# Oujidejihe/PG2024-Data-Parallel-Ray-Tracing

Measured on NVIDIA B200. Metric: Mrays/s, higher is better.
Workload: dtype f32

## Files before the change

include/dprt_types.h:

```cpp
#ifndef DPRT_TYPES_H
#define DPRT_TYPES_H

#include <stdint.h>
#include <stddef.h>

#ifdef __cplusplus
extern "C" {
#endif

#define DPRT_DEFAULT_MAX_COUNT 3
#define DPRT_DEFAULT_SHADOW_PATH_COUNT 4
#define DPRT_EPSILON 1e-3f
#define DPRT_MAX_WORLD 32
#define DPRT_MAX_SCENE_OBJECTS 64
#define DPRT_MAX_LIGHTS 64
#define DPRT_MAX_MATERIALS 256

typedef struct dprt_path_record {
    float    origin[3];
    float    direction[3];
    float    tMax;
    float    throughput[3];
    int32_t  pixelIndex;
    int32_t  shadowPathID;
// ... 127 lines not shown
    int64_t rays_shade;
    int64_t rays_shadow;
    int64_t rays_secondary;
    int64_t nn_queries;
    int64_t paths_sent_offrank;
    int64_t exchange_iters;
    int64_t kernel_launches;
    int64_t bytes_alltoall;
    int64_t rays_shade_cached;
    int64_t rays_walked;
    int64_t walked_traverse;
    int64_t walked_shade;
    int64_t walked_shadow;
    int64_t walked_secondary;
    int64_t paths_partitioned;
} dprt_stats;

enum dprt_buffer_id {
    DPRT_BUF_PATHS = 0,
    DPRT_BUF_TRANSFER = 1,
    DPRT_BUF_TRANSFER_OFFSET = 2,
    DPRT_BUF_DIRECT = 3,
    DPRT_BUF_ENV = 4,
    DPRT_BUF_NN_INPUT = 5,
    DPRT_BUF_NN_QUERY = 6,
    DPRT_BUF_NN_PACKED_INPUT = 7,
    DPRT_BUF_NN_PACKED_QUERY = 8,
    DPRT_BUF_SCENE_OFFSET = 9,
    DPRT_BUF_PRED = 10,
    DPRT_BUF_OCCLUSION = 11,
// ... 49 lines not shown
```

pg2024-data-parallel-ray-tracing_b200/csrc/dprt_api.cu:

```cuda
#include <cuda_runtime.h>
#include <dlfcn.h>
#include <nccl.h>

#include <algorithm>
#include <atomic>
#include <cstdio>
#include <cstring>
#include <memory>
#include <string>
#include <thread>
#include <vector>

#include "dprt.h"
#include "dprt_internal.cuh"
#include "bvh_build.h"
#include "scene_flatten.h"
#include "mlp.cuh"
#include "p2p_exchange.cuh"

using namespace dprt;

struct dprt_bvh8 { Bvh8 b; };

constexpr int kDevStats = 2 + DPRT_STAGE_COUNT;

namespace {

std::string g_create_error;

std::atomic<int> g_streams[64];
int max_connections() {
    const char* e = getenv("CUDA_DEVICE_MAX_CONNECTIONS");
    const int v = e ? atoi(e) : 8;
    return v < 1 ? 1 : (v > 32 ? 32 : v);
}

struct NcclApi {
    void* handle = nullptr;
    ncclResult_t (*GetUniqueId)(ncclUniqueId*) = nullptr;
// ... 102 lines not shown
    P2PPlan* d_plan = nullptr;
    P2PHostPlan* h_plan = nullptr;
    P2PHostPlan* d_hplan = nullptr;
    uint32_t p2pSeq = 0;
    std::vector<void*> ipcOpened;
    int32_t* d_secLive = nullptr;
    int secDirty = 0;
    bool nnScratchDirty = false;
    uint32_t epoch = 1;
    int32_t* d_queue = nullptr;
    cudaStream_t aux = nullptr;
    cudaEvent_t evShade = nullptr, evAux = nullptr;
    int32_t* d_queue_aux = nullptr;
    bool auxPending = false;
    int auxGuardBase = 0;
    float* d_image = nullptr;
    float* d_image_sum = nullptr;
    int32_t* d_gather = nullptr;
    int32_t* h_pinned = nullptr;
    void* d_flush = nullptr; size_t flush_bytes = 0;
    void* d_io = nullptr; size_t io_bytes = 0;
    HitRec* d_rayPark = nullptr; size_t rayParkCount = 0;
    int pathSize = 0, shadowPathSize = 0;
    int sample = 0;
    int queryTotal = 0;
    int queryWhich = 0;
    std::vector<int> h_sceneOffset;
    bool histFresh = false;
    bool qhistFresh = false;
    std::vector<int> h_offsets;
// ... 355 lines not shown
    CK(cudaSetDevice(ctx->device));
    CK(cudaStreamSynchronize(ctx->stream));
    CK(cudaGetLastError());
    return 0;
}
int dprt_get_stats(const dprt_ctx* ctx, dprt_stats* out) {
    if (!ctx || !out) return DPRT_ERR_INVALID;
    *out = ctx->stats;
    if (ctx->d_cacheHits) {
        unsigned long long v[kDevStats] = {0};
        if (cudaSetDevice(ctx->device) != cudaSuccess || cudaStreamSynchronize(ctx->stream) != cudaSuccess ||
            cudaMemcpy(v, ctx->d_cacheHits, sizeof(v), cudaMemcpyDeviceToHost) != cudaSuccess) return DPRT_ERR_CUDA;
        out->rays_shade_cached = (int64_t)v[0]; out->rays_walked = (int64_t)v[1];
        out->walked_traverse = (int64_t)v[2 + DPRT_STAGE_TRAVERSE]; out->walked_shade = (int64_t)v[2 + DPRT_STAGE_SHADE];
        out->walked_shadow = (int64_t)v[2 + DPRT_STAGE_SHADOW_TRACE]; out->walked_secondary = (int64_t)v[2 + DPRT_STAGE_SECONDARY_TRACE];
    }
    return 0;
}
int dprt_reset_stats(dprt_ctx* ctx) {
    if (!ctx) return DPRT_ERR_INVALID;
    ctx->stats = dprt_stats{};
    cudaSetDevice(ctx->device);
    resolve_pending(ctx);
    for (int i = 0; i < DPRT_STAGE_COUNT; i++) { ctx->stageMs[i] = 0.0; ctx->stageLaunches[i] = 0; }
    if (ctx->d_counters) CK(cudaMemsetAsync(ctx->d_counters, 0, 2 * DPRT_STAGE_COUNT * sizeof(unsigned long long), ctx->stream));
    if (ctx->d_cacheHits) CK(cudaMemsetAsync(ctx->d_cacheHits, 0, kDevStats * sizeof(unsigned long long), ctx->stream));
    return 0;
}

int dprt_stage_profile(dprt_ctx* ctx, int enable) {
// ... 350 lines not shown
    if (recv_offset) recv_offset[W] = (int32_t)roff;
    if (recv_total) *recv_total = roff;
    if (all_local) *all_local = offdiag == 0;
    return 0;
}

int dprt_exchange(dprt_ctx* ctx, int* done) {
    if (!ctx) return DPRT_ERR_INVALID;
    CK(cudaSetDevice(ctx->device));
    const int W = ctx->world, me = ctx->rank;
    const size_t R = sizeof(dprt_path_record);
    StageScope sc_(ctx, DPRT_STAGE_EXCHANGE);
    if (W == 1) {
        int r = read_offsets(ctx); if (r) return r;
        const int cnt = ctx->h_offsets[1];
        if (cnt > 0) CK(cudaMemcpyAsync(ctx->hp.paths, ctx->hp.transfer, cnt * R, cudaMemcpyDeviceToDevice, ctx->stream));
        ctx->pathSize = cnt; ctx->stats.paths_partitioned += cnt;
        if (done) *done = 1;
        ctx->stats.exchange_iters++;
        return 0;
    }
    if (!ctx->comm) return fail(ctx, DPRT_ERR_STATE, "dprt_exchange on a multi-rank context without an NCCL communicator");
    NK(g_nccl.AllGather(ctx->hp.transferOffset, ctx->d_gather, W + 1, ncclInt32, ctx->comm, ctx->stream));
    CK(cudaMemcpyAsync(ctx->h_pinned, ctx->d_gather, sizeof(int32_t) * W * (W + 1), cudaMemcpyDeviceToHost, ctx->stream));
    CK(cudaStreamSynchronize(ctx->stream));
    const int32_t* M = ctx->h_pinned;
    ctx->h_offsets.assign(M + me * (W + 1), M + (me + 1) * (W + 1));
    ctx->stats.paths_partitioned += ctx->h_offsets[W];
    std::vector<int32_t> sendCnt(W), recvOff(W + 1, 0), recvCnt(W);
    int64_t recvTotal64 = 0; int allLocal = 0;
    if (dprt_plan_exchange(M, W, me, sendCnt.data(), recvOff.data(), recvCnt.data(), &recvTotal64, &allLocal))
// ... 56 lines not shown
        ctx->stats.exchange_iters++;
    }
    if (done) *done = offdiag == 0;
    return 0;
}

int dprt_shade(dprt_ctx* ctx) {
    if (!ctx) return DPRT_ERR_INVALID;
    CK(cudaSetDevice(ctx->device));
    if (ctx->hp.lightCount < 1) return fail(ctx, DPRT_ERR_STATE, "no lights set");
    ctx->shadowPathSize = ctx->cfg.shadowPathCount * ctx->pathSize;
    const int w = ctx->dirtyIdx == 0 ? 1 : 0;
    ctx->hp.livePixel = ctx->d_live[w]; ctx->liveCount[w] = ctx->pathSize; ctx->shadeIdx = w;
    sync_params(ctx);
    StageScope sc_(ctx, DPRT_STAGE_SHADE, ctx->pathSize > 0);
    launch_shade(ctx->hp, ctx->pathSize, ctx->stream);
    ctx->stats.kernel_launches += trace_kernels_per_stage() * (ctx->pathSize > 0);
    ctx->stats.rays_shade += ctx->pathSize;
    ctx->epoch++;
    ctx->histFresh = false;
    CK(cudaGetLastError());
    return 0;
}

int dprt_reset_nn(dprt_ctx* ctx) {
    if (!ctx) return DPRT_ERR_INVALID;
    CK(cudaSetDevice(ctx->device));
    const bool nnAll = ctx->nnScratchDirty || (ctx->cfg.proxyMode && ctx->dirtyIdx == -2);
    if (nnAll) {
        CK(cudaMemsetAsync(ctx->hp.occlusion, 0, ctx->buf_bytes[DPRT_BUF_OCCLUSION], ctx->stream));
        CK(cudaMemsetAsync(ctx->hp.contribution, 0, ctx->buf_bytes[DPRT_BUF_CONTRIBUTION], ctx->stream));
        ctx->nnScratchDirty = false;
// ... 13 lines not shown
        ctx->stats.kernel_launches += ctx->liveCount[ctx->dirtyIdx] > 0;
    }
    ctx->dirtyIdx = -1;
    CK(cudaMemsetAsync(ctx->hp.queryHist, 0, 64 * sizeof(int32_t), ctx->stream));
    ctx->qhistFresh = false;
    return 0;
}

int dprt_shadow_trace(dprt_ctx* ctx) {
    if (!ctx) return DPRT_ERR_INVALID;
    CK(cudaSetDevice(ctx->device));
    sync_params(ctx);
    CK(cudaMemsetAsync(ctx->hp.queryHist, 0, 64 * sizeof(int32_t), ctx->stream));
    StageScope sc_(ctx, DPRT_STAGE_SHADOW_TRACE, ctx->shadowPathSize > 0);
    launch_shadow_trace(ctx->hp, ctx->shadowPathSize, ctx->stream);
    ctx->stats.kernel_launches += trace_kernels_per_stage() * (ctx->shadowPathSize > 0);
    ctx->stats.rays_shadow += ctx->shadowPathSize;
    if (ctx->shadowPathSize > 0)
        ctx->dirtyIdx = (ctx->shadeIdx >= 0 && (ctx->dirtyIdx == -1 || ctx->dirtyIdx == ctx->shadeIdx)) ? ctx->shadeIdx : -2;
    ctx->qhistFresh = true; ctx->queryWhich = 0;
    CK(cudaGetLastError());
    return 0;
}

int dprt_secondary_trace(dprt_ctx* ctx) {
    if (!ctx) return DPRT_ERR_INVALID;
    CK(cudaSetDevice(ctx->device));
    if (!ctx->cfg.proxyMode) return fail(ctx, DPRT_ERR_STATE, "secondary stage needs proxyMode=1");
    sync_params(ctx);
    CK(cudaMemsetAsync(ctx->hp.queryHist, 0, 64 * sizeof(int32_t), ctx->stream));
    StageScope sc_(ctx, DPRT_STAGE_SECONDARY_TRACE, ctx->pathSize > 0);
// ... 537 lines not shown
    int r;
    if (bounce > 0 && ctx->cfg.proxyMode) {
        if ((r = dprt_reset_nn(ctx))) return r;
        if ((r = dprt_secondary_ray_module(ctx))) return r;
    }
    return 0;
}
int bounce_post(dprt_ctx* ctx) {
    int r;
    if ((r = dprt_shade(ctx))) return r;
    if ((r = dprt_reset_nn(ctx))) return r;
    return dprt_shadow_ray_module(ctx);
}
}

int dprt_render_sample(dprt_ctx* ctx, int sample) {
    if (!ctx) return DPRT_ERR_INVALID;
    int r;
    if ((r = dprt_begin_sample(ctx, sample))) return r;
    if ((r = dprt_path_gen(ctx))) return r;
    const bool overlap = ctx->aux && !ctx->profile;
    for (int bounce = 0; bounce <= ctx->cfg.bounces; bounce++) {
        if ((r = bounce_pre(ctx, bounce))) return r;
        if ((r = dprt_primary_ray_module(ctx))) return r;
        if (!overlap) { if ((r = bounce_post(ctx))) return r; continue; }
        if ((r = join_aux(ctx))) return r;
        if ((r = dprt_shade(ctx))) return r;
        CK(cudaEventRecord(ctx->evShade, ctx->stream));
        cudaStream_t mainStream = ctx->stream; int32_t* mainQueue = ctx->hp.traceQueue;
        ctx->stream = ctx->aux; ctx->hp.traceQueue = ctx->d_queue_aux;
        cudaError_t ce = cudaStreamWaitEvent(ctx->aux, ctx->evShade, 0);
        r = ce != cudaSuccess ? DPRT_ERR_CUDA : dprt_reset_nn(ctx);
        if (!r) r = dprt_shadow_ray_module(ctx);
        if (!r && cudaEventRecord(ctx->evAux, ctx->aux) != cudaSuccess) r = DPRT_ERR_CUDA;
        ctx->stream = mainStream; ctx->hp.traceQueue = mainQueue;
        if (r) return r;
        ctx->auxPending = true; ctx->auxGuardBase = ctx->pathSize;
    }
    return join_aux(ctx);
}

int dprt_render_sample_group(dprt_ctx** ctxs, int W, int sample) {
    if (!ctxs || W < 1) return DPRT_ERR_INVALID;
    int r;
    for (int k = 0; k < W; k++) {
        if ((r = dprt_begin_sample(ctxs[k], sample))) return r;
        if ((r = dprt_path_gen(ctxs[k]))) return r;
    }
    const int bounces = ctxs[0]->cfg.bounces;
    bool deque = true;
    for (int k = 0; k < W; k++) deque = deque && ctxs[k] && deque_enabled(ctxs[k]) && ctxs[k]->world == W && ctxs[k]->rank == k;
    const char* pg = getenv("DPRT_P2P_GROUP");
    bool p2p = deque && W > 1 && W <= 8 && pg && pg[0] == '1';
    if (p2p && !ctxs[0]->p2pGroup) { if ((r = p2p_connect_group(ctxs, W))) return r; }
// ... 274 lines not shown
```

pg2024-data-parallel-ray-tracing_b200/csrc/dprt_internal.cuh:

```cuda
#pragma once
#include <cuda_runtime.h>
#include <stdint.h>
#include "dprt_types.h"
#include "dprt_math.cuh"

namespace dprt {

struct DevObject {
    int32_t nodeID;
    int32_t isProxy;
    float   aabbMin[3];
    float   aabbMax[3];
    float   maxLength;
    float   w2o[12];
    const uint4*  nodes;
    const float4* tris;
    const float*  normals;
};

struct HitRec {
    float   t;
    int32_t prim;
    int32_t tri;
    int32_t obj;
// ... 45 lines not shown
    HitRec*  hitCache;
    uint32_t hitEpoch;
    unsigned long long* cacheHits;
    int32_t  splitL;
    int32_t* secLive;
    int32_t* livePixel;
    const DevTexture* textures;
    const int32_t*    matTex;
    DevTexture        envMap;
    float             envRotation;
};

void launch_path_gen(const DevParams& p, int n, cudaStream_t stream);
void launch_traverse(const DevParams& p, int n, cudaStream_t stream);
void launch_shade(const DevParams& p, int n, cudaStream_t stream);
void launch_shadow_trace(const DevParams& p, int nShadow, cudaStream_t stream);
void launch_secondary_trace(const DevParams& p, int n, cudaStream_t stream);
int trace_kernels_per_stage();
size_t trace_scratch_bytes();
void launch_trace_closest(const DevObject* objects, int sceneSize, const DevTexture* textures, const int32_t* matTex, const dprt_ray* rays,
                          dprt_hit* hits, int64_t n, int32_t* queue, unsigned long long* counters, HitRec* park, cudaStream_t stream);

void launch_train_features(const DevObject* obj, const dprt_ray* rays, const dprt_hit* hits, int64_t n, float* features,
                           float* labels, cudaStream_t stream);

void launch_precom_features(const DevObject* obj, dprt_ray* rays, int64_t n, float* features, float* t_aabb, cudaStream_t stream);
void launch_precom_labels(const DevObject* obj, const dprt_hit* hits, const float* t_aabb, int64_t n, float* labels, uint8_t* valid,
                          cudaStream_t stream);

int spec_texture_sample(const float* rgba, int width, int height, const float* u, const float* v, int64_t n, int clampV, float* out4);
int spec_env_lookup(const float* rgba, int width, int height, float rotationOffset, const float* dirs3, int64_t n, float* out3);
// ... 33 lines not shown
```

pg2024-data-parallel-ray-tracing_b200/csrc/kernels.cu:

```cuda
#include "dprt_internal.cuh"
#include <algorithm>
#include <cstdlib>
#include "bvh_traverse.cuh"

namespace dprt {

namespace {

constexpr int kBlock = 128;

struct PathRegs {
    V3 origin, direction; float tMax; V3 throughput;
    int pixelIndex, shadowPathID; uint32_t visitedMask; int currentNode, targetNode; uint32_t flags;
};
constexpr uint32_t F_SHADOW = 1u, F_DELTA = 1u << 8, F_VALID = 1u << 16, F_HIT = 1u << 24;

DPRT_D PathRegs load_path(const dprt_path_record* p) {
    const float4* q = reinterpret_cast<const float4*>(p);
    float4 a = q[0], b = q[1], c = q[2], d = q[3];
    PathRegs r;
    r.origin = v3(a.x, a.y, a.z); r.direction = v3(a.w, b.x, b.y); r.tMax = b.z;
    r.throughput = v3(b.w, c.x, c.y);
    r.pixelIndex = __float_as_int(c.z); r.shadowPathID = __float_as_int(c.w);
    r.visitedMask = __float_as_uint(d.x); r.currentNode = __float_as_int(d.y);
// ... 84 lines not shown
    const dprt_ray* rays; dprt_hit* rayHits;
    int32_t* hitPrim;
    int32_t* queue;
    unsigned long long* counters;
    int refill;
    int triVote;
    uint32_t prmtMagic;
    uint32_t* coopPool;
    int coop;
    int nodesPerStep;
    HitRec* hitCache; uint32_t epoch; unsigned long long* cacheHits;
    int tailBudget;
    int32_t* parkList;
    HitRec* park;
    const DevTexture* textures; const int32_t* matTex;
};

constexpr int kParkCapacity = 148 * 8 * 128 + 4096;

DPRT_D int next_object(const TraceArgs& a, int from, uint32_t skipMask) {
    for (int k = from; k < a.sceneSize; k++) {
        const DevObject& ob = a.objects[k];
        if (ob.isProxy) continue;
        if ((skipMask >> ob.nodeID) & 1u) continue;
        return k;
    }
    return a.sceneSize;
}


// ... 2 lines not shown
    const bool hit = s.hitTri >= 0;
    if (MODE == TM_TRAVERSE || MODE == TM_SECONDARY || MODE == TM_SHADE) {
        float4* h = reinterpret_cast<float4*>(a.hits + idx);
        h[0] = make_float4(s.tbest, __int_as_float(hit ? s.hitPrim : -1), __int_as_float(s.hitTri), __int_as_float(s.hitObj));
        h[1] = make_float4(s.ha, s.hb, 0.f, 0.f);
    } else if (MODE == TM_SHADOW) {
        if (hit) {
            flags = (flags | F_HIT) & ~F_VALID;
            reinterpret_cast<uint32_t*>(a.recs + idx)[15] = flags;
        }
    } else {
        reinterpret_cast<float2*>(a.rayHits)[idx] = make_float2(s.tbest, __int_as_float(hit ? s.hitPrim : -1));
    }
}

template <int MODE>
DPRT_D bool trace_load_ray(const TraceArgs& a, int my, V3& o, V3& d, float& tmin, float& tmax, uint32_t& flags, uint32_t& skipMask, bool& retry) {
    tmin = DPRT_EPSILON; skipMask = 0u; retry = false; flags = 0u;
    if (MODE == TM_RAYS) {
        const float4 r0 = __ldg(reinterpret_cast<const float4*>(a.rays) + 2 * (size_t)my);
        const float4 r1 = __ldg(reinterpret_cast<const float4*>(a.rays) + 2 * (size_t)my + 1);
        o = v3(r0.x, r0.y, r0.z); tmin = r0.w; d = v3(r1.x, r1.y, r1.z); tmax = r1.w;
        return true;
    }
    const float4* q = reinterpret_cast<const float4*>(a.recs + my);
    const float4 q0 = q[0], q1 = q[1], q3 = q[3];
    o = v3(q0.x, q0.y, q0.z); d = v3(q0.w, q1.x, q1.y); tmax = q1.z;
    flags = __float_as_uint(q3.w);
    if (MODE == TM_TRAVERSE) skipMask = __float_as_uint(q3.x);
    if (MODE == TM_SHADE) {
// ... 2 lines not shown
            tmax = __uint_as_float(__float_as_uint(tmax) + 1u); retry = true;
        } else {
            tmax = FLT_MAX;
        }
    }
    return (flags & F_VALID) != 0u;
}

template <int MODE> constexpr int trace_min_blocks() { return MODE == 2 ? (kTraceBlocksPerSM == 6 ? 7 : kTraceBlocksPerSM) : kTraceBlocksPerSM; }

template <int MODE, bool COUNT>
__global__ void __launch_bounds__(kTraceBlock, trace_min_blocks<MODE>()) trace_kernel(TraceArgs a, int n) {
    constexpr bool ANY = MODE == TM_SHADOW;
    const unsigned FULL = 0xffffffffu;
    __shared__ WarpQueue s_wq[kTraceBlock / 32];
    WarpQueue& w = s_wq[threadIdx.x >> 5];
    const int lane = threadIdx.x & 31;
    const TexCtx tc = {a.textures, a.matTex};
    Trav s;
    uint2 stack[DPRT_STACK];
    int idx = -1, obj = 0, pend = 0;
    bool exh = false;
    uint32_t skipMask = 0u, flags = 0u;
    bool retry = false;
    uint32_t cached = 0u;
    uint32_t walked = 0u;
    TraceCount cnt = {0u, 0u};
    bool exhausted = false;
    int qlen = 0;
#if DPRT_TAIL_PARK
    int tail = 0;
// ... 51 lines not shown
                }
            }
        }
        const unsigned act = __ballot_sync(FULL, idx >= 0);
        if (act == 0u) { if (exhausted) break; continue; }

        const int minBusy = exhausted ? 1 : (32 - kRefill + 1);
        do {
#if DPRT_TAIL_PARK
            const bool parkNow = exhausted && a.tailBudget > 0 && ++tail > a.tailBudget;
            if (parkNow) { while (qlen > 0) tri_round<ANY, COUNT>(w, qlen, lane, s, obj, pend, cnt, tc); }
#else
            constexpr bool parkNow = false;
#endif
            if (!parkNow) wq_append(w, qlen, lane, idx >= 0, s, pend);
            if (idx >= 0) {
                bool done = false;
                if (obj >= a.sceneSize) {
                    done = pend == 0;
                } else {
                    if (!exh && s.tg.y == 0u && (s.ng.y & 0xff000000u) == 0u) {
                        if (s.sp == 0) exh = true; else s.ng = stack[--s.sp];
                    }
                    if (ANY && s.hitTri >= 0) { exh = true; s.tg.y = 0u; }
                    if (exh && s.tg.y == 0u && pend == 0) {
                        if (ANY && s.hitTri >= 0) done = true;
                        else {
                            obj = next_object(a, obj + 1, skipMask);
                            if (obj < a.sceneSize) {
                                trav_enter_object(s, a.objects[obj].nodes, a.objects[obj].tris); wq_set_object(w, lane, s); exh = false;
                            } else done = true;
                        }
                    }
                }
                if (done && MODE == TM_SHADE && retry && s.hitTri < 0) {
                    retry = false; done = false;
                    s.tbest = FLT_MAX;
                    obj = next_object(a, 0, 0u);
                    if (obj < a.sceneSize) {
                        trav_enter_object(s, a.objects[obj].nodes, a.objects[obj].tris); wq_set_object(w, lane, s); exh = false;
                    } else done = true;
                }
                if (done) {
                    trace_end<MODE>(a, idx, s, flags);
                    idx = -1;
                }
            }
#if DPRT_TAIL_PARK
            if (parkNow) {
                const bool mine = idx >= 0;
                const unsigned pm = __ballot_sync(FULL, mine);
                if (pm != 0u) {
                    int pbase = 0;
                    if (lane == __ffs(pm) - 1) pbase = atomicAdd(a.queue + 1, __popc(pm));
                    pbase = __shfl_sync(FULL, pbase, __ffs(pm) - 1);
                    if (mine) {
                        a.parkList[pbase + __popc(pm & ((1u << lane) - 1u))] = idx;
                        if (!ANY) {
                            float4* h = reinterpret_cast<float4*>(a.park + idx);
                            h[0] = make_float4(s.tbest, __int_as_float(s.hitPrim), __int_as_float(s.hitTri), __int_as_float(s.hitObj));
// ... 18 lines not shown
            const unsigned nodeM = __ballot_sync(FULL, canNode);
            const unsigned waitM = __ballot_sync(FULL, busy && !canNode);
            if (qlen > 0 && (qlen >= 32 || nodeM == 0u || __popc(waitM) >= a.triVote)) tri_round<ANY, COUNT>(w, qlen, lane, s, obj, pend, cnt, tc);
            else if (canNode) {
                int left = a.nodesPerStep;
#pragma unroll 1
                for (;;) {
                    const uint32_t tm = trav_node<COUNT>(s, stack, cnt, a.prmtMagic);
                    if (s.tg.y != 0u) { w.tmask[lane] = tm; break; }
                    if (--left == 0) break;
                    if ((s.ng.y & 0xff000000u) == 0u) { if (s.sp == 0) break; s.ng = stack[--s.sp]; }
                }
            }
        } while (__popc(__ballot_sync(FULL, idx >= 0)) >= minBusy);
    }
    if (a.cacheHits) {
        if (MODE == TM_SHADE) {
            cached = __reduce_add_sync(FULL, cached);
            if (lane == 0 && cached) atomicAdd(a.cacheHits, (unsigned long long)cached);
        }
        walked = __reduce_add_sync(FULL, walked);
        if (lane == 0 && walked) { atomicAdd(a.cacheHits + 1, (unsigned long long)walked); atomicAdd(a.cacheHits + 2 + StageOf<MODE>::id, (unsigned long long)walked); }
    }
    if (COUNT) {
        if (cnt.nodes) atomicAdd(a.counters + 2 * StageOf<MODE>::id, (unsigned long long)cnt.nodes);
        if (cnt.tris) atomicAdd(a.counters + 2 * StageOf<MODE>::id + 1, (unsigned long long)cnt.tris);
    }
}

#if DPRT_TAIL_PARK
// ... 42 lines not shown
                    if (resume) { s.tlimit = tlimit; s.tiePrim = (s.hitTri >= 0 && s.hitObj == obj) ? s.hitPrim : 0x7fffffff; }
                    wq_set_object(w, 0, s);
                }
                resume = false;
                __syncwarp();
                coop_run<ANY, COUNT>(w, pool, qlen, lane, 0, s, stack, obj, pend, exh, cnt, a.prmtMagic, tc);
                if (ANY && __shfl_sync(FULL, (int)(s.hitTri >= 0), 0)) break;
                obj = next_object(a, obj + 1, skipMask);
            }
            const bool again = MODE == TM_SHADE && retry && !__shfl_sync(FULL, (int)(s.hitTri >= 0), 0);
            if (!again) break;
            retry = false;
            if (lane == 0) s.tbest = FLT_MAX;
            obj = next_object(a, 0, 0u);
        }
        if (lane == 0) trace_end<MODE>(a, idx, s, flags);
        __syncwarp();
    }
    if (COUNT) {
        if (cnt.nodes) atomicAdd(a.counters + 2 * StageOf<MODE>::id, (unsigned long long)cnt.nodes);
        if (cnt.tris) atomicAdd(a.counters + 2 * StageOf<MODE>::id + 1, (unsigned long long)cnt.tris);
    }
}
#endif

DPRT_D void merge_trace_result(const DevParams& p, int i, PathRegs& path) {
    const float4 h0 = reinterpret_cast<const float4*>(p.hits + i)[0];
    const int prim = __float_as_int(h0.y);
    if (prim < 0) return;
    path.tMax = h0.x; path.currentNode = p.worldID; path.flags |= F_HIT;
    if (p.hitPrim) p.hitPrim[i] = prim;
// ... 75 lines not shown
    if (xi1 < fr) {
        wi = v3(-wo.x, -wo.y, wo.z);
        const float cosTheta = fabsf(wi.z);
        const float thr = cosTheta == 0.0f ? 0.0f : fr / cosTheta;
        s.wiLocal = wi; s.weight = thr / fr;
    } else {
        const float ft = 1.0f - fr;
        const float cosTheta = fabsf(wi.z);
        const float thr = cosTheta == 0.0f ? 0.0f : ft / cosTheta;
        const float corr = (etaI / etaT) * (etaI / etaT);
        s.wiLocal = wi; s.weight = thr * corr / ft;
    }
    return s;
}

__global__ void __launch_bounds__(kBlock) shade_post_kernel(DevParams p, int n) {
    const int i = blockIdx.x * blockDim.x + threadIdx.x;
    if (i == 0) { p.traceQueue[0] = 0; p.traceQueue[1] = 0; p.traceQueue[2] = 0; }
    if (i >= n) return;
    PathRegs path = load_path(p.paths + i);
    if (!(path.flags & F_VALID)) { if (p.livePixel) p.livePixel[i] = -1; return; }
    const V3 o = path.origin, d = path.direction;
    const float4 h0 = reinterpret_cast<const float4*>(p.hits + i)[0], h1 = reinterpret_cast<const float4*>(p.hits + i)[1];
    const float ht = h0.x; const int hprim = __float_as_int(h0.y), htri = __float_as_int(h0.z), hobj = __float_as_int(h0.w);
    const bool isHit = htri >= 0;
    if (p.hitPrim) p.hitPrim[i] = isHit ? hprim : -1;
    if (p.livePixel) p.livePixel[i] = isHit ? path.pixelIndex : -1;
    if (!isHit) {
        add_env(p, path);
        store_zero_path(p.paths + i);
        for (int s = 0; s < p.spc; s++) store_zero_path(p.paths + (size_t)i * p.spc + s + p.pathSize);
        return;
    }
    const DevObject& ob = p.objects[hobj];
    const float4 tb = __ldg(ob.tris + 3 * (size_t)htri + 1);
    const int matID = __float_as_int(tb.w);
    const dprt_material mat = p.materials[matID];
    V3 albedo = v3(mat.baseColor[0], mat.baseColor[1], mat.baseColor[2]);
// ... 149 lines not shown
    return addedDirect ? -1 : count;
}

DPRT_D void flush_query_hist(const DevParams& p, const int* shHist) {
    const int t = threadIdx.x;
    if (t < p.sceneSize) { if (shHist[t]) atomicAdd(p.queryHist + t, shHist[t]); }
    else if (t >= 32 && t < 32 + p.sceneSize) { if (shHist[t]) atomicAdd(p.queryHist + p.sceneSize + (t - 32), shHist[t]); }
}

__global__ void __launch_bounds__(kBlock) shadow_post_kernel(DevParams p, int nShadow) {
    __shared__ int shHist[64];
    if (threadIdx.x < 64) shHist[threadIdx.x] = 0;
    __syncthreads();
    const int i = blockIdx.x * blockDim.x + threadIdx.x;
    if (i == 0) { p.traceQueue[0] = 0; p.traceQueue[1] = 0; p.traceQueue[2] = 0; }
    if (i < nShadow && p.proxyMode == 0) {
        const float4* q = reinterpret_cast<const float4*>(p.paths + (size_t)p.pathSize + i);
        const float4 q3 = q[3];
        if (__float_as_uint(q3.w) & F_VALID) {
            const float4 q2 = q[2];
            const float tx = q[1].w;
            const size_t px = ((size_t)p.frameBufferSize * __float_as_int(q2.w) + __float_as_int(q2.z)) * 3;
            const float inv = (float)p.spc;
            p.direct[px + 0] += tx / inv;
            p.direct[px + 1] += q2.x / inv;
            p.direct[px + 2] += q2.y / inv;
        }
    } else if (i < nShadow) {
        const PathRegs path = load_path(p.paths + (size_t)p.pathSize + i);
        if (!(path.flags & F_VALID)) {
            clear_query_slots(p, i, 0);
        } else {
            const int r = proxy_march<false>(p, path, i, path.tMax, shHist);
            if (r < 0) {
                const size_t px = ((size_t)p.frameBufferSize * path.shadowPathID + path.pixelIndex) * 3;
                const float inv = (float)p.spc;
                p.direct[px + 0] += path.throughput.x / inv;
                p.direct[px + 1] += path.throughput.y / inv;
                p.direct[px + 2] += path.throughput.z / inv;
            }
        }
    }
    __syncthreads();
// ... 124 lines not shown
        if (a.counters) trace_finish_kernel<MODE, true><<<blocks, kTraceBlock, 0, s>>>(a);
        else trace_finish_kernel<MODE, false><<<blocks, kTraceBlock, 0, s>>>(a);
    }
#endif
    if (MODE == TM_RAYS) cudaMemsetAsync(a.queue, 0, 3 * sizeof(int32_t), s);
}

TraceArgs trace_args(const DevParams& p, dprt_path_record* recs) {
    TraceArgs a;
    a.objects = p.objects; a.sceneSize = p.sceneSize; a.worldID = p.worldID; a.recs = recs; a.hits = p.hits;
    a.rays = nullptr; a.rayHits = nullptr; a.hitPrim = p.hitPrim; a.queue = p.traceQueue; a.counters = p.counters;
    a.refill = tune_refill(); a.triVote = tune_trivote(); a.prmtMagic = 0x47000000u; a.coop = tune_coop(); a.nodesPerStep = tune_nodes();
    a.hitCache = p.hitCache; a.epoch = p.hitEpoch; a.cacheHits = p.cacheHits;
    a.tailBudget = tune_tail(); a.parkList = nullptr; a.park = p.hits;
    a.textures = p.textures; a.matTex = p.matTex;
    return a;
}

}

int spec_texture_sample(const float* rgba, int width, int height, const float* u, const float* v, int64_t n, int clampV, float* out4) {
    if (!rgba || !u || !v || !out4 || width < 1 || height < 1 || n < 0) return DPRT_ERR_INVALID;
    const DevTexture T = {reinterpret_cast<const float4*>(rgba), width, height};
    for (int64_t i = 0; i < n; i++) {
        const float4 c = tex_bilinear(T, u[i], v[i], clampV != 0);
        out4[4 * i + 0] = c.x; out4[4 * i + 1] = c.y; out4[4 * i + 2] = c.z; out4[4 * i + 3] = c.w;
    }
    return 0;
}
int spec_env_lookup(const float* rgba, int width, int height, float rotationOffset, const float* dirs3, int64_t n, float* out3) {
// ... 23 lines not shown
    if (e == cudaSuccess) e = cudaFuncGetAttributes(&fa, traverse_post_kernel);
    return e;
}

void launch_path_gen(const DevParams& p, int n, cudaStream_t s) {
    if (n > 0) path_gen_kernel<<<blocks_for(n), kBlock, 0, s>>>(p, n);
}
void launch_traverse(const DevParams& p, int n, cudaStream_t s) {
    if (n <= 0) return;
    launch_trace<TM_TRAVERSE>(trace_args(p, p.paths), n, s);
    traverse_post_kernel<<<blocks_for(n), kBlock, 0, s>>>(p, n);
}
void launch_shade(const DevParams& p, int n, cudaStream_t s) {
    if (n <= 0) return;
    launch_trace<TM_SHADE>(trace_args(p, p.paths), n, s);
    shade_post_kernel<<<blocks_for(n), kBlock, 0, s>>>(p, n);
}
void launch_shadow_trace(const DevParams& p, int nShadow, cudaStream_t s) {
    if (nShadow <= 0) return;
    launch_trace<TM_SHADOW>(trace_args(p, p.paths + p.pathSize), nShadow, s);
    shadow_post_kernel<<<blocks_for(nShadow), kBlock, 0, s>>>(p, nShadow);
}
void launch_secondary_trace(const DevParams& p, int n, cudaStream_t s) {
    if (n <= 0) return;
    launch_trace<TM_SECONDARY>(trace_args(p, p.paths), n, s);
    secondary_post_kernel<<<blocks_for(n), kBlock, 0, s>>>(p, n);
}
void launch_train_features(const DevObject* obj, const dprt_ray* rays, const dprt_hit* hits, int64_t n, float* features,
                           float* labels, cudaStream_t s) {
    if (n > 0) train_features_kernel<<<blocks_for(n), kBlock, 0, s>>>(obj, rays, hits, n, features, labels);
}
void launch_precom_features(const DevObject* obj, dprt_ray* rays, int64_t n, float* features, float* t_aabb, cudaStream_t s) {
    if (n > 0) precom_features_kernel<<<blocks_for(n), kBlock, 0, s>>>(obj, rays, n, features, t_aabb);
}
void launch_precom_labels(const DevObject* obj, const dprt_hit* hits, const float* t_aabb, int64_t n, float* labels, uint8_t* valid, cudaStream_t s) {
    if (n > 0) precom_label_kernel<<<blocks_for(n), kBlock, 0, s>>>(obj, hits, t_aabb, n, labels, valid);
}
// ... 15 lines not shown
```

pg2024-data-parallel-ray-tracing_b200/ctypes_defs.py:

```python
import ctypes as C

import numpy as np

DPRT_EPSILON = 1e-3
MAX_WORLD = 32


class Config(C.Structure):
    _fields_ = [("width", C.c_int32), ("height", C.c_int32), ("spp", C.c_int32), ("bounces", C.c_int32),
                ("shadowPathCount", C.c_int32), ("maxCount", C.c_int32), ("sceneSize", C.c_int32),
                ("proxyMode", C.c_int32), ("pathGenMode", C.c_int32), ("mlpDtype", C.c_int32),
                ("envColor", C.c_float * 3), ("mainRayRetrace", C.c_int32), ("serialStages", C.c_int32),
                ("referenceMigrate", C.c_int32)]


class ObjectDesc(C.Structure):
    _fields_ = [("nodeID", C.c_int32), ("isProxy", C.c_int32), ("aabbMin", C.c_float * 3), ("aabbMax", C.c_float * 3),
                ("maxLength", C.c_float), ("worldToObject", C.c_float * 12)]


class Camera(C.Structure):
    _fields_ = [("origin", C.c_float * 3), ("U", C.c_float * 3), ("V", C.c_float * 3), ("W", C.c_float * 3),
                ("width", C.c_int32), ("height", C.c_int32)]

# ... 37 lines not shown
        else:
            md[k].texCoords, md[k].nTexCoords, md[k].texCoordIndices = None, 0, None
        md[k].materialID = int(m["material"])
    ins = (InstanceDesc * len(instances))()
    for k, (mi, M) in enumerate(instances):
        ins[k].mesh = int(mi)
        ins[k].objectToWorld[:] = np.asarray(M, np.float32).reshape(12).tolist()
    return md, len(meshes), ins, len(instances), keep


class Stats(C.Structure):
    _fields_ = [("rays_traverse", C.c_int64), ("rays_shade", C.c_int64), ("rays_shadow", C.c_int64),
                ("rays_secondary", C.c_int64), ("nn_queries", C.c_int64), ("paths_sent_offrank", C.c_int64),
                ("exchange_iters", C.c_int64), ("kernel_launches", C.c_int64), ("bytes_alltoall", C.c_int64),
                ("rays_shade_cached", C.c_int64), ("rays_walked", C.c_int64), ("walked_traverse", C.c_int64),
                ("walked_shade", C.c_int64), ("walked_shadow", C.c_int64), ("walked_secondary", C.c_int64), ("paths_partitioned", C.c_int64)]

    def as_dict(self):
        return {k: int(getattr(self, k)) for k, _ in self._fields_ if k != "reserved_"}


PATH_DTYPE = np.dtype([("origin", "<f4", 3), ("direction", "<f4", 3), ("tMax", "<f4"), ("throughput", "<f4", 3),
                       ("pixelIndex", "<i4"), ("shadowPathID", "<i4"), ("visitedMask", "<u4"), ("currentNode", "<i4"),
                       ("targetNode", "<i4"), ("isShadowRay", "u1"), ("isDelta", "u1"), ("isValid", "u1"), ("isHit", "u1")])
QUERY_DTYPE = np.dtype([("throughput", "<f4", 3), ("pixelIndex", "<i4"), ("hitSequence", "<i4"), ("hitAABBID", "<i4"),
                        ("shadowPathID", "<i4"), ("instanceID", "<i4"), ("pathIndex", "<i4"), ("normalizedT", "<f4"),
                        ("isValid", "u1"), ("isInside", "u1"), ("pad_", "u1", 2), ("reserved_", "<i4")])
RAY_DTYPE = np.dtype([("origin", "<f4", 3), ("tMin", "<f4"), ("direction", "<f4", 3), ("tMax", "<f4")])
HIT_DTYPE = np.dtype([("t", "<f4"), ("primID", "<i4")])
MATERIAL_DTYPE = np.dtype([("baseColor", "<f4", 3), ("bsdfType", "<i4")])
LIGHT_DTYPE = np.dtype([("p0", "<f4", 3), ("p1", "<f4", 3), ("p2", "<f4", 3), ("Le", "<f4", 3)])
NODE_DTYPE = np.dtype([("p", "<f4", 3), ("e", "u1", 3), ("imask", "u1"), ("childBase", "<u4"), ("triBase", "<u4"),
                       ("tmask", "<u4"), ("reserved_", "<u4"), ("qlox", "u1", 8), ("qloy", "u1", 8), ("qloz", "u1", 8),
                       ("qhix", "u1", 8), ("qhiy", "u1", 8), ("qhiz", "u1", 8)])
TRI_DTYPE = np.dtype([("v0", "<f4", 3), ("primID", "<i4"), ("v1", "<f4", 3), ("matID", "<i4"), ("v2", "<f4", 3), ("pad_", "<i4")])

assert PATH_DTYPE.itemsize == 64 and QUERY_DTYPE.itemsize == 48 and RAY_DTYPE.itemsize == 32 and HIT_DTYPE.itemsize == 8
assert NODE_DTYPE.itemsize == 80 and TRI_DTYPE.itemsize == 48 and MATERIAL_DTYPE.itemsize == 16 and LIGHT_DTYPE.itemsize == 48
assert C.sizeof(Config) == 64 and C.sizeof(ObjectDesc) == 84 and C.sizeof(Camera) == 56 and C.sizeof(Stats) == 128
assert C.sizeof(MeshDesc) == 88 and C.sizeof(InstanceDesc) == 56

P2P_HANDLE_BYTES = 208

BUF_PATHS, BUF_TRANSFER, BUF_TRANSFER_OFFSET, BUF_DIRECT, BUF_ENV, BUF_NN_INPUT, BUF_NN_QUERY, BUF_NN_PACKED_INPUT, \
    BUF_NN_PACKED_QUERY, BUF_SCENE_OFFSET, BUF_PRED, BUF_OCCLUSION, BUF_CONTRIBUTION, BUF_HIT_PRIM = range(14)

STAGE_NAMES = ("path_gen", "traverse", "partition", "exchange", "shade", "shadow_trace", "secondary_trace", "bucket",
               "proxy_mlp", "frame_update", "depth_update", "target_update", "image", "trace_closest")
STAGE_COUNT = len(STAGE_NAMES)

BUFFER_DTYPES = {
    BUF_PATHS: PATH_DTYPE, BUF_TRANSFER: PATH_DTYPE, BUF_TRANSFER_OFFSET: np.dtype("<i4"), BUF_DIRECT: np.dtype("<f4"),
    BUF_ENV: np.dtype("<f4"), BUF_NN_INPUT: np.dtype("<u2"), BUF_NN_QUERY: QUERY_DTYPE, BUF_NN_PACKED_INPUT: np.dtype("<u2"),
    BUF_NN_PACKED_QUERY: QUERY_DTYPE, BUF_SCENE_OFFSET: np.dtype("<i4"), BUF_PRED: np.dtype("<u2"),
# ... 48 lines not shown
```

Baseline: 2587.

## Skip shade re-trace via hit cache on single rank; fuse shadow direct accumulation

On a single rank with no proxies, the exchange step no longer copies partitioned records back into the paths buffer. Shading then reads them straight from the transfer buffer and takes its hits from the per-pixel hit cache, so the shade trace kernel is skipped, and stale cache entries are counted. Separately, the shadow trace kernel now adds direct lighting for unoccluded shadow rays itself, with warp-batched flushes, so the separate shadow post kernel is dropped outside proxy mode. This relies on the hit cache staying valid for shading, and the in-kernel direct accumulation uses non-atomic += just as the old post kernel did.

```diff
diff --git a/include/dprt_types.h b/include/dprt_types.h
--- a/include/dprt_types.h
+++ b/include/dprt_types.h
@@ -165,6 +165,7 @@
     int64_t walked_shadow;
     int64_t walked_secondary;
     int64_t paths_partitioned;
+    int64_t shade_cache_stale;
 } dprt_stats;
 
 enum dprt_buffer_id {
diff --git a/pg2024-data-parallel-ray-tracing_b200/csrc/dprt_api.cu b/pg2024-data-parallel-ray-tracing_b200/csrc/dprt_api.cu
--- a/pg2024-data-parallel-ray-tracing_b200/csrc/dprt_api.cu
+++ b/pg2024-data-parallel-ray-tracing_b200/csrc/dprt_api.cu
@@ -5,6 +5,7 @@
 #include <algorithm>
 #include <atomic>
 #include <cstdio>
+#include <cstdlib>
 #include <cstring>
 #include <memory>
 #include <string>
@@ -22,7 +23,7 @@
 
 struct dprt_bvh8 { Bvh8 b; };
 
-constexpr int kDevStats = 2 + DPRT_STAGE_COUNT;
+constexpr int kDevStats = 3 + DPRT_STAGE_COUNT;
 
 namespace {
 
@@ -155,6 +156,8 @@
     int32_t* d_queue_aux = nullptr;
     bool auxPending = false;
     int auxGuardBase = 0;
+    bool shortcut = false;
+    bool recsInTransfer = false;
     float* d_image = nullptr;
     float* d_image_sum = nullptr;
     int32_t* d_gather = nullptr;
@@ -540,6 +543,7 @@
         out->rays_shade_cached = (int64_t)v[0]; out->rays_walked = (int64_t)v[1];
         out->walked_traverse = (int64_t)v[2 + DPRT_STAGE_TRAVERSE]; out->walked_shade = (int64_t)v[2 + DPRT_STAGE_SHADE];
         out->walked_shadow = (int64_t)v[2 + DPRT_STAGE_SHADOW_TRACE]; out->walked_secondary = (int64_t)v[2 + DPRT_STAGE_SECONDARY_TRACE];
+        out->shade_cache_stale = (int64_t)v[2 + DPRT_STAGE_COUNT];
     }
     return 0;
 }
@@ -920,7 +924,8 @@
     if (W == 1) {
         int r = read_offsets(ctx); if (r) return r;
         const int cnt = ctx->h_offsets[1];
-        if (cnt > 0) CK(cudaMemcpyAsync(ctx->hp.paths, ctx->hp.transfer, cnt * R, cudaMemcpyDeviceToDevice, ctx->stream));
+        if (ctx->shortcut) ctx->recsInTransfer = true;
+        else if (cnt > 0) CK(cudaMemcpyAsync(ctx->hp.paths, ctx->hp.transfer, cnt * R, cudaMemcpyDeviceToDevice, ctx->stream));
         ctx->pathSize = cnt; ctx->stats.paths_partitioned += cnt;
         if (done) *done = 1;
         ctx->stats.exchange_iters++;
@@ -1007,8 +1012,11 @@
     ctx->hp.livePixel = ctx->d_live[w]; ctx->liveCount[w] = ctx->pathSize; ctx->shadeIdx = w;
     sync_params(ctx);
     StageScope sc_(ctx, DPRT_STAGE_SHADE, ctx->pathSize > 0);
-    launch_shade(ctx->hp, ctx->pathSize, ctx->stream);
-    ctx->stats.kernel_launches += trace_kernels_per_stage() * (ctx->pathSize > 0);
+    const bool cached = ctx->recsInTransfer;
+    ctx->recsInTransfer = false;
+    if (cached) launch_shade_cached(ctx->hp, ctx->pathSize, ctx->stream);
+    else launch_shade(ctx->hp, ctx->pathSize, ctx->stream);
+    ctx->stats.kernel_launches += (cached ? 1 : trace_kernels_per_stage()) * (ctx->pathSize > 0);
     ctx->stats.rays_shade += ctx->pathSize;
     ctx->epoch++;
     ctx->histFresh = false;
@@ -1052,7 +1060,7 @@
     CK(cudaMemsetAsync(ctx->hp.queryHist, 0, 64 * sizeof(int32_t), ctx->stream));
     StageScope sc_(ctx, DPRT_STAGE_SHADOW_TRACE, ctx->shadowPathSize > 0);
     launch_shadow_trace(ctx->hp, ctx->shadowPathSize, ctx->stream);
-    ctx->stats.kernel_launches += trace_kernels_per_stage() * (ctx->shadowPathSize > 0);
+    ctx->stats.kernel_launches += shadow_trace_kernels(ctx->hp) * (ctx->shadowPathSize > 0);
     ctx->stats.rays_shadow += ctx->shadowPathSize;
     if (ctx->shadowPathSize > 0)
         ctx->dirtyIdx = (ctx->shadeIdx >= 0 && (ctx->dirtyIdx == -1 || ctx->dirtyIdx == ctx->shadeIdx)) ? ctx->shadeIdx : -2;
@@ -1620,8 +1628,15 @@
 }
 }
 
-int dprt_render_sample(dprt_ctx* ctx, int sample) {
-    if (!ctx) return DPRT_ERR_INVALID;
+namespace {
+bool single_rank_shortcut(const dprt_ctx* ctx) {
+    if (ctx->world != 1 || ctx->cfg.proxyMode || !ctx->d_hitCache || ctx->hp.hitPrim) return false;
+    for (const ObjectHost& o : ctx->objects) if (o.present && o.desc.isProxy) return false;
+    const char* v = getenv("DPRT_SINGLE_RANK_SHORTCUT");
+    return !(v && std::strcmp(v, "0") == 0);
+}
+
+int render_sample(dprt_ctx* ctx, int sample) {
     int r;
     if ((r = dprt_begin_sample(ctx, sample))) return r;
     if ((r = dprt_path_gen(ctx))) return r;
@@ -1644,6 +1659,15 @@
         ctx->auxPending = true; ctx->auxGuardBase = ctx->pathSize;
     }
     return join_aux(ctx);
+}
+}
+
+int dprt_render_sample(dprt_ctx* ctx, int sample) {
+    if (!ctx) return DPRT_ERR_INVALID;
+    ctx->shortcut = single_rank_shortcut(ctx);
+    const int r = render_sample(ctx, sample);
+    ctx->shortcut = false; ctx->recsInTransfer = false;
+    return r;
 }
 
 int dprt_render_sample_group(dprt_ctx** ctxs, int W, int sample) {
diff --git a/pg2024-data-parallel-ray-tracing_b200/csrc/dprt_internal.cuh b/pg2024-data-parallel-ray-tracing_b200/csrc/dprt_internal.cuh
--- a/pg2024-data-parallel-ray-tracing_b200/csrc/dprt_internal.cuh
+++ b/pg2024-data-parallel-ray-tracing_b200/csrc/dprt_internal.cuh
@@ -83,7 +83,9 @@
 void launch_path_gen(const DevParams& p, int n, cudaStream_t stream);
 void launch_traverse(const DevParams& p, int n, cudaStream_t stream);
 void launch_shade(const DevParams& p, int n, cudaStream_t stream);
+void launch_shade_cached(const DevParams& p, int n, cudaStream_t stream);
 void launch_shadow_trace(const DevParams& p, int nShadow, cudaStream_t stream);
+int shadow_trace_kernels(const DevParams& p);
 void launch_secondary_trace(const DevParams& p, int n, cudaStream_t stream);
 int trace_kernels_per_stage();
 size_t trace_scratch_bytes();
diff --git a/pg2024-data-parallel-ray-tracing_b200/csrc/kernels.cu b/pg2024-data-parallel-ray-tracing_b200/csrc/kernels.cu
--- a/pg2024-data-parallel-ray-tracing_b200/csrc/kernels.cu
+++ b/pg2024-data-parallel-ray-tracing_b200/csrc/kernels.cu
@@ -122,6 +122,7 @@
     int32_t* parkList;
     HitRec* park;
     const DevTexture* textures; const int32_t* matTex;
+    float* direct; int frameBufferSize; int spc;
 };
 
 constexpr int kParkCapacity = 148 * 8 * 128 + 4096;
@@ -154,6 +155,23 @@
     }
 }
 
+DPRT_D void shadow_add_direct(const TraceArgs& a, int rec) {
+    const float4* q = reinterpret_cast<const float4*>(a.recs + rec);
+    const float tx = q[1].w;
+    const float4 q2 = q[2];
+    const size_t px = ((size_t)a.frameBufferSize * __float_as_int(q2.w) + __float_as_int(q2.z)) * 3;
+    const float inv = (float)a.spc;
+    a.direct[px + 0] += tx / inv;
+    a.direct[px + 1] += q2.x / inv;
+    a.direct[px + 2] += q2.y / inv;
+}
+
+DPRT_D void shadow_flush(const TraceArgs& a, const int32_t* lits, int nlit, int lane) {
+    __syncwarp();
+    for (int k = lane; k < nlit; k += 32) shadow_add_direct(a, lits[k]);
+    __syncwarp();
+}
+
 template <int MODE>
 DPRT_D bool trace_load_ray(const TraceArgs& a, int my, V3& o, V3& d, float& tmin, float& tmax, uint32_t& flags, uint32_t& skipMask, bool& retry) {
     tmin = DPRT_EPSILON; skipMask = 0u; retry = false; flags = 0u;
@@ -186,7 +204,10 @@
     constexpr bool ANY = MODE == TM_SHADOW;
     const unsigned FULL = 0xffffffffu;
     __shared__ WarpQueue s_wq[kTraceBlock / 32];
+    __shared__ int32_t s_lits[ANY ? kTraceBlock / 32 * 64 : 1];
     WarpQueue& w = s_wq[threadIdx.x >> 5];
+    int32_t* lits = s_lits + (ANY ? (threadIdx.x >> 5) * 64 : 0);
+    int nlit = 0;
     const int lane = threadIdx.x & 31;
     const TexCtx tc = {a.textures, a.matTex};
     Trav s;
@@ -268,6 +289,7 @@
             constexpr bool parkNow = false;
 #endif
             if (!parkNow) wq_append(w, qlen, lane, idx >= 0, s, pend);
+            int lit = -1;
             if (idx >= 0) {
                 bool done = false;
                 if (obj >= a.sceneSize) {
@@ -297,7 +319,16 @@
                 }
                 if (done) {
                     trace_end<MODE>(a, idx, s, flags);
+                    if (ANY && s.hitTri < 0) lit = idx;
                     idx = -1;
+                }
+            }
+            if (ANY && a.direct) {
+                const unsigned lm = __ballot_sync(FULL, lit >= 0);
+                if (lm != 0u) {
+                    if (lit >= 0) lits[nlit + __popc(lm & ((1u << lane) - 1u))] = lit;
+                    nlit += __popc(lm);
+                    if (nlit >= 32) { shadow_flush(a, lits, nlit, lane); nlit = 0; }
                 }
             }
 #if DPRT_TAIL_PARK
@@ -346,6 +377,7 @@
             }
         } while (__popc(__ballot_sync(FULL, idx >= 0)) >= minBusy);
     }
+    if (ANY && nlit > 0) shadow_flush(a, lits, nlit, lane);
     if (a.cacheHits) {
         if (MODE == TM_SHADE) {
             cached = __reduce_add_sync(FULL, cached);
@@ -418,7 +450,10 @@
             if (lane == 0) s.tbest = FLT_MAX;
             obj = next_object(a, 0, 0u);
         }
-        if (lane == 0) trace_end<MODE>(a, idx, s, flags);
+        if (lane == 0) {
+            trace_end<MODE>(a, idx, s, flags);
+            if (ANY && a.direct && s.hitTri < 0) shadow_add_direct(a, idx);
+        }
         __syncwarp();
     }
     if (COUNT) {
@@ -524,14 +559,23 @@
     return s;
 }
 
-__global__ void __launch_bounds__(kBlock) shade_post_kernel(DevParams p, int n) {
+__global__ void __launch_bounds__(kBlock) shade_post_kernel(DevParams p, int n, const dprt_path_record* src, bool fromCache) {
     const int i = blockIdx.x * blockDim.x + threadIdx.x;
     if (i == 0) { p.traceQueue[0] = 0; p.traceQueue[1] = 0; p.traceQueue[2] = 0; }
     if (i >= n) return;
-    PathRegs path = load_path(p.paths + i);
+    PathRegs path = load_path(src + i);
     if (!(path.flags & F_VALID)) { if (p.livePixel) p.livePixel[i] = -1; return; }
     const V3 o = path.origin, d = path.direction;
-    const float4 h0 = reinterpret_cast<const float4*>(p.hits + i)[0], h1 = reinterpret_cast<const float4*>(p.hits + i)[1];
+    const float4* hr = reinterpret_cast<const float4*>(fromCache ? p.hitCache + path.pixelIndex : p.hits + i);
+    const float4 h0 = hr[0], h1 = hr[1];
+    if (fromCache) {
+        const unsigned m = __activemask();
+        const unsigned stale = __ballot_sync(m, __float_as_uint(h1.z) != p.hitEpoch);
+        if ((threadIdx.x & 31) == __ffs(m) - 1) {
+            if (m != stale) atomicAdd(p.cacheHits, (unsigned long long)__popc(m & ~stale));
+            if (stale) atomicAdd(p.cacheHits + 2 + DPRT_STAGE_COUNT, (unsigned long long)__popc(stale));
+        }
+    }
     const float ht = h0.x; const int hprim = __float_as_int(h0.y), htri = __float_as_int(h0.z), hobj = __float_as_int(h0.w);
     const bool isHit = htri >= 0;
     if (p.hitPrim) p.hitPrim[i] = isHit ? hprim : -1;
@@ -711,19 +755,7 @@
     __syncthreads();
     const int i = blockIdx.x * blockDim.x + threadIdx.x;
     if (i == 0) { p.traceQueue[0] = 0; p.traceQueue[1] = 0; p.traceQueue[2] = 0; }
-    if (i < nShadow && p.proxyMode == 0) {
-        const float4* q = reinterpret_cast<const float4*>(p.paths + (size_t)p.pathSize + i);
-        const float4 q3 = q[3];
-        if (__float_as_uint(q3.w) & F_VALID) {
-            const float4 q2 = q[2];
-            const float tx = q[1].w;
-            const size_t px = ((size_t)p.frameBufferSize * __float_as_int(q2.w) + __float_as_int(q2.z)) * 3;
-            const float inv = (float)p.spc;
-            p.direct[px + 0] += tx / inv;
-            p.direct[px + 1] += q2.x / inv;
-            p.direct[px + 2] += q2.y / inv;
-        }
-    } else if (i < nShadow) {
+    if (i < nShadow) {
         const PathRegs path = load_path(p.paths + (size_t)p.pathSize + i);
         if (!(path.flags & F_VALID)) {
             clear_query_slots(p, i, 0);
@@ -878,6 +910,7 @@
     a.hitCache = p.hitCache; a.epoch = p.hitEpoch; a.cacheHits = p.cacheHits;
     a.tailBudget = tune_tail(); a.parkList = nullptr; a.park = p.hits;
     a.textures = p.textures; a.matTex = p.matTex;
+    a.direct = nullptr; a.frameBufferSize = p.frameBufferSize; a.spc = p.spc;
     return a;
 }
 
@@ -931,13 +964,20 @@
 void launch_shade(const DevParams& p, int n, cudaStream_t s) {
     if (n <= 0) return;
     launch_trace<TM_SHADE>(trace_args(p, p.paths), n, s);
-    shade_post_kernel<<<blocks_for(n), kBlock, 0, s>>>(p, n);
+    shade_post_kernel<<<blocks_for(n), kBlock, 0, s>>>(p, n, p.paths, false);
+}
+void launch_shade_cached(const DevParams& p, int n, cudaStream_t s) {
+    if (n > 0) shade_post_kernel<<<blocks_for(n), kBlock, 0, s>>>(p, n, p.transfer, true);
 }
 void launch_shadow_trace(const DevParams& p, int nShadow, cudaStream_t s) {
     if (nShadow <= 0) return;
-    launch_trace<TM_SHADOW>(trace_args(p, p.paths + p.pathSize), nShadow, s);
-    shadow_post_kernel<<<blocks_for(nShadow), kBlock, 0, s>>>(p, nShadow);
-}
+    TraceArgs a = trace_args(p, p.paths + p.pathSize);
+    if (!p.proxyMode) a.direct = p.direct;
+    launch_trace<TM_SHADOW>(a, nShadow, s);
+    if (p.proxyMode) shadow_post_kernel<<<blocks_for(nShadow), kBlock, 0, s>>>(p, nShadow);
+    else cudaMemsetAsync(p.traceQueue, 0, 3 * sizeof(int32_t), s);
+}
+int shadow_trace_kernels(const DevParams& p) { return trace_kernels_per_stage() - (p.proxyMode ? 0 : 1); }
 void launch_secondary_trace(const DevParams& p, int n, cudaStream_t s) {
     if (n <= 0) return;
     launch_trace<TM_SECONDARY>(trace_args(p, p.paths), n, s);
diff --git a/pg2024-data-parallel-ray-tracing_b200/ctypes_defs.py b/pg2024-data-parallel-ray-tracing_b200/ctypes_defs.py
--- a/pg2024-data-parallel-ray-tracing_b200/ctypes_defs.py
+++ b/pg2024-data-parallel-ray-tracing_b200/ctypes_defs.py
@@ -75,7 +75,8 @@
                 ("rays_secondary", C.c_int64), ("nn_queries", C.c_int64), ("paths_sent_offrank", C.c_int64),
                 ("exchange_iters", C.c_int64), ("kernel_launches", C.c_int64), ("bytes_alltoall", C.c_int64),
                 ("rays_shade_cached", C.c_int64), ("rays_walked", C.c_int64), ("walked_traverse", C.c_int64),
-                ("walked_shade", C.c_int64), ("walked_shadow", C.c_int64), ("walked_secondary", C.c_int64), ("paths_partitioned", C.c_int64)]
+                ("walked_shade", C.c_int64), ("walked_shadow", C.c_int64), ("walked_secondary", C.c_int64), ("paths_partitioned", C.c_int64),
+                ("shade_cache_stale", C.c_int64)]
 
     def as_dict(self):
         return {k: int(getattr(self, k)) for k, _ in self._fields_ if k != "reserved_"}
@@ -98,7 +99,7 @@
 
 assert PATH_DTYPE.itemsize == 64 and QUERY_DTYPE.itemsize == 48 and RAY_DTYPE.itemsize == 32 and HIT_DTYPE.itemsize == 8
 assert NODE_DTYPE.itemsize == 80 and TRI_DTYPE.itemsize == 48 and MATERIAL_DTYPE.itemsize == 16 and LIGHT_DTYPE.itemsize == 48
-assert C.sizeof(Config) == 64 and C.sizeof(ObjectDesc) == 84 and C.sizeof(Camera) == 56 and C.sizeof(Stats) == 128
+assert C.sizeof(Config) == 64 and C.sizeof(ObjectDesc) == 84 and C.sizeof(Camera) == 56 and C.sizeof(Stats) == 136
 assert C.sizeof(MeshDesc) == 88 and C.sizeof(InstanceDesc) == 56
 
 P2P_HANDLE_BYTES = 208
```

After: 2778 (median of 6 runs). 1.07x the previous value.
